# mapbox/robosat

Measured on AMD Instinct MI355X. Metric: 512x512 tiles/sec train+predict, 1/2/4/8 MI355X; mIoU vs CPU ref, higher is better.
Workload: dtype f32; 1 GPU; rs predict ResNet50-UNet, bs=16 3x512x512 fp32 per GPU, 2 classes (BASELINE configs[1]); parallelism=tiles sharded over 1 rank(s), no collective

## Files before the change

robosat_amd/csrc/conv_wino33_f32.hip:

```cpp
#define RS_CONV_INSTANTIATE
#include "conv_igemm_dma_kernel.h"
#include "final_head.h"

namespace {

struct Wino33Args {
  const float* src;
  const float* u;
  const float* scale;
  const float* shift;
  float* out;
  int N, H, W, Cin, Cout;
  int BBY, BBX;
  int nsub;
  int ncb;
  int relu;
  const float* hw;
  const float* hb;
  const double* hanchors;
  float* hout;
  unsigned char* hq;
  int hC, hmode, hov;
  float* stats;
  const float* mask;
  const unsigned char* mask_bits;
  const float* bn_y;
  const float* bn_mean;
  const float* bn_invstd;
};

typedef float f32x2 __attribute__((ext_vector_type(2)));
__device__ __forceinline__ f32x2 pk_add(f32x2 a, f32x2 b) {
  f32x2 d;
  asm("v_pk_add_f32 %0, %1, %2" : "=v"(d) : "v"(a), "v"(b));
  return d;
}
__device__ __forceinline__ f32x2 pk_sub(f32x2 a, f32x2 b) {
  f32x2 d;
  asm("v_pk_add_f32 %0, %1, %2 neg_lo:[0,1] neg_hi:[0,1]" : "=v"(d) : "v"(a), "v"(b));
  return d;
}
constexpr int kPB = 8, kHW = 2 * kPB + 2, kPITCH = kHW, kHALF = kHW / 2;
constexpr int kSBROWS = (kHW * kPITCH + 7) / 8 * 8;

__device__ __forceinline__ int w33_lane_tile(int l) { return (l & 1) | (((l >> 1) & 1) << 2) | (((l >> 2) & 1) << 1) | (l & 8); }
__device__ __forceinline__ int w33_swz(int row) { return (row ^ (row >> 1)) & 3; }

template <int TG, int CG, int MODE = 0>
__global__ __launch_bounds__(512, 1) void conv_wino33_f32_kernel(const Wino33Args p) {
  constexpr int HEAD = (MODE >= 1 && MODE <= 3) ? MODE : 0;
  constexpr bool BWD = MODE == 5;
  constexpr bool STATS = MODE == 4 || BWD;
  constexpr int NW = TG * CG;
  static_assert(NW == 8, "8 waves");
  static_assert(!HEAD || (TG == 4 && CG == 2), "the fused head: one 8x8 patch of tiles x all 32 couts per block");
  constexpr int BMT = 16 * TG, BN = 16 * CG;
  constexpr int SB = BMT / (kPB * kPB);
  static_assert(SB * kPB * kPB == BMT, "whole sub-blocks per block");
  constexpr int AROWS = SB * kSBROWS;
  constexpr int IA = (AROWS + 15) / 16, IB = 16 * BN / 16;
  constexpr int AROWS_PAD = IA * 16;
  constexpr int NI = (IA + IB + NW - 1) / NW;
  constexpr int STAGE = (AROWS_PAD + 16 * BN) * 64;
  constexpr int KC = 16;

  constexpr int HEADW = kHeadMaxC * 32 + kHeadMaxC, XROW = 4 * kHeadMaxC + 4, XCH = BMT * XROW;
  constexpr int XST = 2 * TG * BN;
  __shared__ __attribute__((aligned(16))) unsigned char smem[2 * STAGE + 2 * AROWS_PAD * 4 + (HEAD ? (HEADW + 2 * XCH) * 4 : 0) + (STATS ? 2 * XST * 4 : 0)];
  int* tabs = reinterpret_cast<int*>(smem + 2 * STAGE);
  float* hws = reinterpret_cast<float*>(smem + 2 * STAGE + 2 * AROWS_PAD * 4);
  float* xch = hws + HEADW;
  float* xst = reinterpret_cast<float*>(smem + 2 * STAGE + 2 * AROWS_PAD * 4);

  const int tid = threadIdx.x, lane = tid & 63;
  const int wave = __builtin_amdgcn_readfirstlane(tid >> 6);
  const int tg = wave % TG, cg = wave / TG;
  const int per_img = p.BBY * p.BBX;
  const int nk = p.Cin / KC;
  const int ntiles = ((p.nsub + SB - 1) / SB) * p.ncb;
  const int first = rs_xcd_remap(blockIdx.x, gridDim.x);
  const int nitems = (ntiles - first + (int)gridDim.x - 1) / (int)gridDim.x;
  const unsigned int lds0 = __builtin_amdgcn_readfirstlane(rs_lds_addr(smem));
  const long img = (long)p.H * p.W * p.Cin;

  auto decode = [&](int it, int& mblk, int& nblk) __attribute__((always_inline)) {
    mblk = it / p.ncb;
    nblk = it - mblk * p.ncb;
  };
  auto build_table = [&](int seq) __attribute__((always_inline)) {
    int mblk, nblk;
    decode(first + seq * (int)gridDim.x, mblk, nblk);
    const int sub0 = mblk * SB, nfirst = sub0 / per_img;
    int* tab = tabs + (seq & 1) * AROWS_PAD;
    for (int rho = tid; rho < AROWS_PAD; rho += 64 * NW) {
      int v = -1;
      if (rho < AROWS) {
        const int sb = rho / kSBROWS, rem = rho - sb * kSBROWS;
        const int hy = rem / kPITCH, xs = rem - hy * kPITCH;
        const int hx = hy >= kHW ? -1 : (xs < kHALF ? 2 * xs : 2 * (xs - kHALF) + 1);
        const int sub = sub0 + sb;
        if (hx >= 0 && sub < p.nsub) {
          const int n = sub / per_img, r2 = sub - n * per_img;
          const int bby = r2 / p.BBX, bbx = r2 - bby * p.BBX;
          const int y = 2 * bby * kPB - 1 + hy, x = 2 * bbx * kPB - 1 + hx;
          if ((unsigned)y < (unsigned)p.H && (unsigned)x < (unsigned)p.W) v = ((n - nfirst) * p.H + y) * p.W + x;
        }
      }
      tab[rho] = v;
    }
    rs_lds_writes_done();
  };

  const int ra = lane >> 2, pp = lane & 3;
  int doff[NI];
  int f_seq = 0, f_kc = 0, f_g = 0;
  __amdgpu_buffer_rsrc_t rsrc = rs_dma_rsrc<kDmaClamp>(p.src, 0);
  const __amdgpu_buffer_rsrc_t rsrcu = rs_dma_rsrc<kDmaClamp>(p.u, (long)16 * p.Cout * p.Cin * 4);
  auto fetch_item = [&]() __attribute__((always_inline)) {
    int mblk, nblk;
    decode(first + f_seq * (int)gridDim.x, mblk, nblk);
    const int nfirst = __builtin_amdgcn_readfirstlane((mblk * SB) / per_img);
    rsrc = rs_dma_rsrc<kDmaClamp>(p.src + nfirst * img, (long)(p.N - nfirst) * img * 4);
    const int* tab = tabs + (f_seq & 1) * AROWS_PAD;
#pragma unroll
    for (int j = 0; j < NI; ++j) {
      const int ii = wave + NW * j;
      if (ii < IA) {
        const int rho = 16 * ii + ra;
        const int pix = tab[rho];
        doff[j] = pix < 0 ? kDmaOOB : pix * (p.Cin * 4) + ((pp ^ w33_swz(rho)) & 3) * 16;
      } else {
        const int w = 16 * (ii - IA) + ra;
        const int xi = w / BN, co = w - xi * BN;
        doff[j] = ((xi * p.Cout + nblk * BN + co) * p.Cin) * 4 + ((pp ^ w33_swz(w)) & 3) * 16;
      }
    }
  };
  auto fetch_chunk = [&](auto interleave, bool past) __attribute__((always_inline)) {
    if (!past && f_kc == 0) fetch_item();
    const unsigned int fL = lds0 + (f_g & 1) * STAGE;
    const int fs = f_kc * KC * 4;
    interleave([&](int j) __attribute__((always_inline)) {
      const int ii = wave + NW * j;
      if (ii < IA) rs_dma16(rsrc, fL + ii * 1024, doff[j], fs);
      else if (ii < IA + IB) rs_dma16(rsrcu, fL + ii * 1024, doff[j], fs);
    });
    ++f_g;
    if (!past && ++f_kc == nk) {
      f_kc = 0;
      ++f_seq;
    }
  };

  const int l15 = lane & 15, pc = lane >> 4;
  const int t = 16 * tg + w33_lane_tile(l15);
  const int tsb = t / (kPB * kPB), tq = t - tsb * (kPB * kPB);
  const int tty = tq / kPB, ttx = tq - tty * kPB;
  int addrA[4][4];
  {
    const int rho0 = tsb * kSBROWS + 2 * tty * kPITCH + ttx;
#pragma unroll
    for (int r = 0; r < 4; ++r)
#pragma unroll
      for (int c = 0; c < 4; ++c) {
        const int rho = rho0 + r * kPITCH + (c >> 1) + (c & 1) * kHALF;
        addrA[r][c] = rho * 64 + ((pc ^ w33_swz(rho)) & 3) * 16;
      }
  }
  const int addrB = AROWS_PAD * 64 + (16 * cg + l15) * 64 + ((pc ^ w33_swz(l15)) & 3) * 16;

  if constexpr (HEAD) {
    for (int f = threadIdx.x; f < HEADW; f += 64 * NW) {
      const int c = f < kHeadMaxC * 32 ? f / 32 : f - kHeadMaxC * 32;
      hws[f] = c >= p.hC ? 0.f : (f < kHeadMaxC * 32 ? p.hw[f] : (p.hb ? p.hb[c] : 0.f));
    }
  }
  build_table(0);
  __syncthreads();
  fetch_chunk([&](auto issue) __attribute__((always_inline)) {
#pragma unroll
    for (int j = 0; j < NI; ++j) issue(j);
  }, false);
  const int total = nitems * nk;

  float hmine[kHeadMaxC];
  long hpix = -1;
  int hbuf = 0;
  auto finish_head = [&]() __attribute__((always_inline)) {
    if constexpr (HEAD) {
      if (cg == 0) {
        const float* xrow = xch + hbuf * XCH + (16 * tg + l15) * XROW + pc * kHeadMaxC;
        const f32x4 o0 = *reinterpret_cast<const f32x4*>(xrow), o1 = *reinterpret_cast<const f32x4*>(xrow + 4);
        float lg[kHeadMaxC];
#pragma unroll
        for (int c = 0; c < kHeadMaxC; ++c) lg[c] = (hmine[c] + (c < 4 ? o0[c] : o1[c - 4])) + hws[kHeadMaxC * 32 + c];
        if (hpix >= 0)
          rs_final_epilogue_rt(lg, p.hC, hpix, (long)p.H * p.W, HEAD == 1 ? (p.hmode & 1) : HEAD, p.hanchors, p.hq, p.hout, p.W, p.hov);
      }
    }
  };

  int st_buf = 0, st_row = 0, st_col = 0;
  auto finish_stats = [&]() __attribute__((always_inline)) {
    if constexpr (STATS) {
      if ((!BWD || p.stats) && threadIdx.x < 2 * BN) {
        const int which = threadIdx.x / BN, c = threadIdx.x - which * BN;
        const float* x = xst + st_buf * XST + which * TG * BN + c;
        float a = 0.f;
#pragma unroll
        for (int t = 0; t < TG; ++t) a += x[t * BN];
        p.stats[((long)st_row * 2 + which) * p.Cout + st_col + c] = a;
      }
    }
  };
  int g = 0;
  for (int seq = 0; seq < nitems; ++seq) {
    f32x4 acc[16];
#pragma unroll
    for (int x = 0; x < 16; ++x) acc[x] = f32x4{0.f, 0.f, 0.f, 0.f};

    for (int kc = 0; kc < nk; ++kc, ++g) {
      rs_dma_wait();
      __syncthreads();
      if (HEAD && kc == 0 && seq > 0) finish_head();
      if (STATS && kc == 0 && seq > 0) finish_stats();
      const unsigned char* L = smem + (g & 1) * STAGE;
      f32x4 V[16];
      {
        f32x2 Pl[4][4], Ph[4][4];
#pragma unroll
        for (int r = 0; r < 4; ++r)
#pragma unroll
          for (int c = 0; c < 4; ++c) {
            const f32x4 q = *reinterpret_cast<const f32x4*>(L + addrA[r][c]);
            Pl[r][c] = f32x2{q[0], q[1]};
            Ph[r][c] = f32x2{q[2], q[3]};
          }
        f32x2 Tl[4][4], Th[4][4];
#pragma unroll
        for (int r = 0; r < 4; ++r) {
          Tl[r][0] = pk_sub(Pl[r][0], Pl[r][2]);
          Tl[r][1] = pk_add(Pl[r][1], Pl[r][2]);
          Tl[r][2] = pk_sub(Pl[r][2], Pl[r][1]);
          Tl[r][3] = pk_sub(Pl[r][1], Pl[r][3]);
          Th[r][0] = pk_sub(Ph[r][0], Ph[r][2]);
          Th[r][1] = pk_add(Ph[r][1], Ph[r][2]);
          Th[r][2] = pk_sub(Ph[r][2], Ph[r][1]);
          Th[r][3] = pk_sub(Ph[r][1], Ph[r][3]);
        }
#pragma unroll
        for (int c = 0; c < 4; ++c) {
          const f32x2 l0 = pk_sub(Tl[0][c], Tl[2][c]), l1 = pk_add(Tl[1][c], Tl[2][c]), l2 = pk_sub(Tl[2][c], Tl[1][c]), l3 = pk_sub(Tl[1][c], Tl[3][c]);
          const f32x2 h0 = pk_sub(Th[0][c], Th[2][c]), h1 = pk_add(Th[1][c], Th[2][c]), h2 = pk_sub(Th[2][c], Th[1][c]), h3 = pk_sub(Th[1][c], Th[3][c]);
          V[0 * 4 + c] = f32x4{l0[0], l0[1], h0[0], h0[1]};
          V[1 * 4 + c] = f32x4{l1[0], l1[1], h1[0], h1[1]};
          V[2 * 4 + c] = f32x4{l2[0], l2[1], h2[0], h2[1]};
          V[3 * 4 + c] = f32x4{l3[0], l3[1], h3[0], h3[1]};
        }
      }
      const bool more = g + 1 < total;
      constexpr int NMMA = 64, PSTEP = NMMA / NI >= 1 ? NMMA / NI : 1;
      f32x4 Bq[16];
      Bq[0] = *reinterpret_cast<const f32x4*>(L + addrB);
      __builtin_amdgcn_sched_barrier(0);
      auto mfmas = [&](auto issue) __attribute__((always_inline)) {
#pragma unroll
        for (int x = 0; x < 16; ++x) {
          if (x + 1 < 16) {
            Bq[x + 1] = *reinterpret_cast<const f32x4*>(L + addrB + (x + 1) * BN * 64);
            __builtin_amdgcn_sched_barrier(0);
          }
#pragma unroll
          for (int k = 0; k < 4; ++k) {
            const int q = x * 4 + k;
            if (q % PSTEP == 0 && q / PSTEP < NI) issue(q / PSTEP);
            acc[x] = __builtin_amdgcn_mfma_f32_16x16x4f32(Bq[x][k], V[x][k], acc[x], 0, 0, 0);
          }
        }
      };
      fetch_chunk([&](auto issue) __attribute__((always_inline)) { mfmas(issue); }, !more);
      if (kc == 0 && seq + 1 < nitems) build_table(seq + 1);
    }

    int mblk, nblk;
    decode(first + seq * (int)gridDim.x, mblk, nblk);
    const int sub = mblk * SB + tsb;
    const bool live = sub < p.nsub;
    const int n = sub / per_img, r2 = sub - n * per_img;
    const int bby = r2 / p.BBX, bbx = r2 - bby * p.BBX;
    const int a0 = 2 * (bby * kPB + tty), b0 = 2 * (bbx * kPB + ttx);
    const int co = nblk * BN + 16 * cg + 4 * pc;
    f32x4 Y[2][2];
    if (live || HEAD) {
      f32x4 sc = {1.f, 1.f, 1.f, 1.f}, sh = {0.f, 0.f, 0.f, 0.f};
      if (p.scale) sc = *reinterpret_cast<const f32x4*>(p.scale + co);
      if (p.shift) sh = *reinterpret_cast<const f32x4*>(p.shift + co);
      f32x4 R[2][4];
#pragma unroll
      for (int b = 0; b < 4; ++b) {
        R[0][b] = (acc[0 * 4 + b] + acc[1 * 4 + b]) + acc[2 * 4 + b];
        R[1][b] = (acc[1 * 4 + b] - acc[2 * 4 + b]) - acc[3 * 4 + b];
      }
#pragma unroll
      for (int u = 0; u < 2; ++u)
#pragma unroll
        for (int v = 0; v < 2; ++v) {
          f32x4 y = v == 0 ? (R[u][0] + R[u][1]) + R[u][2] : (R[u][1] - R[u][2]) - R[u][3];
          y = y * sc + sh;
          if (p.relu) {
#pragma unroll
            for (int e = 0; e < 4; ++e) y[e] = fmaxf(y[e], 0.f);
          }
          Y[u][v] = y;
        }
    }
    if constexpr (!HEAD) {
      f32x4 s0 = {0.f, 0.f, 0.f, 0.f}, s1 = {0.f, 0.f, 0.f, 0.f};
      if (live) {
        if constexpr (BWD) {
          long o[4];
          bool ok[4];
          f32x4 zm[4], yv[4];
          unsigned int bits[4];
#pragma unroll
          for (int q = 0; q < 4; ++q) {
            const int a = a0 + (q >> 1), b = b0 + (q & 1);
            ok[q] = a < p.H && b < p.W;
            o[q] = ok[q] ? ((long)(n * p.H + a) * p.W + b) * p.Cout + co : (long)co;
          }
          if (p.mask) {
#pragma unroll
            for (int q = 0; q < 4; ++q) zm[q] = *reinterpret_cast<const f32x4*>(p.mask + o[q]);
          }
          if (p.mask_bits) {
#pragma unroll
            for (int q = 0; q < 4; ++q) bits[q] = p.mask_bits[o[q] >> 3];
          }
          f32x4 mu = {0.f, 0.f, 0.f, 0.f}, is = mu;
          if (p.stats) {
#pragma unroll
            for (int q = 0; q < 4; ++q) yv[q] = *reinterpret_cast<const f32x4*>(p.bn_y + o[q]);
            mu = *reinterpret_cast<const f32x4*>(p.bn_mean + co);
            is = *reinterpret_cast<const f32x4*>(p.bn_invstd + co);
          }
#pragma unroll
          for (int q = 0; q < 4; ++q) {
            f32x4 y = Y[q >> 1][q & 1];
            if (p.mask) {
#pragma unroll
              for (int e = 0; e < 4; ++e) y[e] = zm[q][e] > 0.f ? y[e] : 0.f;
            }
            if (p.mask_bits) {
              const unsigned int nib = bits[q] >> (o[q] & 4);
#pragma unroll
              for (int e = 0; e < 4; ++e) y[e] = ((nib >> e) & 1u) ? y[e] : 0.f;
            }
            if (!ok[q]) continue;
            *reinterpret_cast<f32x4*>(p.out + o[q]) = y;
            if (p.stats) {
              s0 += y;
              s1 += y * ((yv[q] - mu) * is);
            }
          }
        } else {
#pragma unroll
          for (int u = 0; u < 2; ++u)
#pragma unroll
            for (int v = 0; v < 2; ++v) {
              const int a = a0 + u, b = b0 + v;
              if (a >= p.H || b >= p.W) continue;
              *reinterpret_cast<f32x4*>(p.out + ((long)(n * p.H + a) * p.W + b) * p.Cout + co) = Y[u][v];
              if constexpr (STATS) {
                s0 += Y[u][v];
                s1 += Y[u][v] * Y[u][v];
              }
            }
        }
      }
      if constexpr (STATS) {
        if (!BWD || p.stats) {
#pragma unroll
          for (int e = 0; e < 4; ++e) {
            s0[e] = rs_row16_sum(s0[e]);
            s1[e] = rs_row16_sum(s1[e]);
          }
          st_buf = seq & 1;
          st_row = mblk;
          st_col = nblk * BN;
          if (l15 == 0) {
            float* x = xst + st_buf * XST + tg * BN + 16 * cg + 4 * pc;
            *reinterpret_cast<f32x4*>(x) = s0;
            *reinterpret_cast<f32x4*>(x + TG * BN) = s1;
            rs_lds_writes_done();
          }
        }
      }
    } else {
      float part[4][kHeadMaxC];
#pragma unroll
      for (int c = 0; c < kHeadMaxC; ++c) {
        if (c < p.hC) {
          const f32x4 wv = *reinterpret_cast<const f32x4*>(hws + c * 32 + 16 * cg + 4 * pc);
#pragma unroll
          for (int px = 0; px < 4; ++px) {
            const f32x4 y = Y[px >> 1][px & 1];
            float v = fmaf(y[3], wv[3], fmaf(y[2], wv[2], fmaf(y[1], wv[1], y[0] * wv[0])));
            v = rs_xor32_sum(rs_xor16_sum(v));
            part[px][c] = v;
          }
        } else {
#pragma unroll
          for (int px = 0; px < 4; ++px) part[px][c] = 0.f;
        }
      }
      hbuf = seq & 1;
      if (cg == 1 && pc == 0) {
        float* xrow = xch + hbuf * XCH + (16 * tg + l15) * XROW;
#pragma unroll
        for (int px = 0; px < 4; ++px) {
          *reinterpret_cast<f32x4*>(xrow + px * kHeadMaxC) = f32x4{part[px][0], part[px][1], part[px][2], part[px][3]};
          *reinterpret_cast<f32x4*>(xrow + px * kHeadMaxC + 4) = f32x4{part[px][4], part[px][5], part[px][6], part[px][7]};
        }
        rs_lds_writes_done();
      }
#pragma unroll
      for (int c = 0; c < kHeadMaxC; ++c) hmine[c] = pc == 0 ? part[0][c] : (pc == 1 ? part[1][c] : (pc == 2 ? part[2][c] : part[3][c]));
      const int a = a0 + (pc >> 1), b = b0 + (pc & 1);
      hpix = (live && a < p.H && b < p.W) ? (long)(n * p.H + a) * p.W + b : -1;
    }
  }
  if constexpr (HEAD) {
    __syncthreads();
    if (nitems > 0) finish_head();
  }
  if constexpr (STATS) {
    __syncthreads();
    if (nitems > 0) finish_stats();
  }
  rs_dma_wait();
}

__global__ void pack_wino33_weight_kernel(const float* __restrict__ w, float* __restrict__ u, int Cout, int Cin, long total) {
  const long i = (long)blockIdx.x * blockDim.x + threadIdx.x;
  if (i >= total) return;
  const int ci = (int)(i % Cin), co = (int)(i / Cin);
  const float* g = w + (long)co * 9 * Cin + ci;
  float gg[3][3];
#pragma unroll
  for (int r = 0; r < 3; ++r)
#pragma unroll
    for (int c = 0; c < 3; ++c) gg[r][c] = g[(long)(r * 3 + c) * Cin];
  float t[4][3];
#pragma unroll
  for (int c = 0; c < 3; ++c) {
    t[0][c] = gg[0][c];
    t[1][c] = 0.5f * ((gg[0][c] + gg[1][c]) + gg[2][c]);
    t[2][c] = 0.5f * ((gg[0][c] - gg[1][c]) + gg[2][c]);
    t[3][c] = gg[2][c];
  }
#pragma unroll
  for (int r = 0; r < 4; ++r) {
    const float v[4] = {t[r][0], 0.5f * ((t[r][0] + t[r][1]) + t[r][2]), 0.5f * ((t[r][0] - t[r][1]) + t[r][2]), t[r][2]};
#pragma unroll
    for (int c = 0; c < 4; ++c) u[((long)(r * 4 + c) * Cout + co) * Cin + ci] = v[c];
  }
}

int w33_plan(const rs_conv_desc* d, int* cgroups) {
  if (!d || d->N <= 0 || d->Hs <= 0 || d->Ws <= 0 || d->C1 < 32 || (d->C1 % 16) || d->C2 != 0 || d->Cout <= 0 || (d->Cout % 16)) return 0;
  if (!(d->ups == 0 && d->kh == 3 && d->kw == 3 && d->stride == 1 && d->pad == 1 && d->Ho == d->Hs && d->Wo == d->Ws && !d->stem)) return 0;
  if ((d->Hs + 1) / 2 < kPB || (d->Ws + 1) / 2 < kPB) return 0;
  *cgroups = (d->Cout % 32 == 0) ? 2 : 1;
  const int sb = 16 * (8 / *cgroups) / (kPB * kPB);
  if ((long)(sb + 1) * d->Hs * d->Ws * d->C1 * 4 >= (1L << 31)) return 0;
  if ((long)16 * d->Cout * d->C1 * 4 >= (1L << 31)) return 0;
  if ((long)d->N * d->Ho * d->Wo * d->Cout >= (1L << 62)) return 0;
  return 1;
}

}

extern "C" int rs_conv2d_wino33_ok(const rs_conv_desc* d) {
  int cgn;
  return w33_plan(d, &cgn);
}

extern "C" const char* rs_conv2d_wino33_name(const rs_conv_desc* d) {
  int cgn;
  if (!w33_plan(d, &cgn)) return "";
  return cgn == 2 ? "conv_wino_f32<3x3,p8,64x32>" : "conv_wino_f32<3x3,p8,128x16>";
}

extern "C" int rs_conv2d_wino33_head_ok(const rs_conv_desc* d, int C) {
  int cgn;
  return w33_plan(d, &cgn) && cgn == 2 && d->Cout == 32 && C >= 1 && C <= kHeadMaxC;
}

extern "C" const char* rs_conv2d_wino33_head_name(void) { return "conv_wino_f32<3x3+final,p8,64x32>"; }

extern "C" int rs_pack_wino33_weight(const float* w_krsc, float* u, int Cout, int Cin, rs_stream_t stream) {
  if (!w_krsc || !u || Cout <= 0 || Cin <= 0) return RS_EINVAL;
  const long total = (long)Cout * Cin;
  pack_wino33_weight_kernel<<<rs_cdiv(total, 256), 256, 0, (hipStream_t)stream>>>(w_krsc, u, Cout, Cin, total);
  return RS_LAUNCH_RESULT();
}

extern "C" int rs_conv2d_fwd_wino33(const rs_conv_desc* d, const float* src, const float* u, const float* scale, const float* shift,
                                    float* out, rs_stream_t stream) {
  int cgn;
  if (!w33_plan(d, &cgn) || !src || !u || !out) return RS_EINVAL;
  Wino33Args a;
  a.src = src;
  a.u = u;
  a.scale = scale;
  a.shift = shift;
  a.out = out;
  a.N = d->N;
  a.H = d->Hs;
  a.W = d->Ws;
  a.Cin = d->C1;
  a.Cout = d->Cout;
  a.BBY = rs_cdiv((d->Hs + 1) / 2, kPB);
  a.BBX = rs_cdiv((d->Ws + 1) / 2, kPB);
  a.nsub = d->N * a.BBY * a.BBX;
  a.ncb = d->Cout / (16 * cgn);
  a.relu = d->relu;
  a.hw = a.hb = nullptr;
  a.hanchors = nullptr;
  a.hout = nullptr;
  a.hq = nullptr;
  a.hC = a.hmode = a.hov = 0;
  a.stats = nullptr;
  a.mask = a.bn_y = a.bn_mean = a.bn_invstd = nullptr;
  a.mask_bits = nullptr;
  const int sb = 16 * (8 / cgn) / (kPB * kPB);
  const long items = (long)rs_cdiv(a.nsub, sb) * a.ncb;
  if (items >= (1L << 31)) return RS_EINVAL;
  const int grid = (int)(items < rs_cu_count() ? items : rs_cu_count());
  hipStream_t s = (hipStream_t)stream;
  if (cgn == 2) conv_wino33_f32_kernel<4, 2><<<grid, 512, 0, s>>>(a);
  else conv_wino33_f32_kernel<8, 1><<<grid, 512, 0, s>>>(a);
  return RS_LAUNCH_RESULT();
}

extern "C" int rs_conv2d_fwd_wino33_head(const rs_conv_desc* d, const float* src, const float* u, const float* scale, const float* shift,
                                         const float* final_w, const float* final_b, int C, int mode, const double* anchors,
                                         int overlap, float* out, uint8_t* qout, rs_stream_t stream) {
  if (!rs_conv2d_wino33_head_ok(d, C) || !src || !u || !final_w || mode < 0 || mode > 3) return RS_EINVAL;
  if (mode <= 1 ? !out : !qout) return RS_EINVAL;
  if (mode == 2 && (!anchors || C < 2 || overlap < 0 || 2 * overlap >= d->Hs || 2 * overlap >= d->Ws)) return RS_EINVAL;
  if (mode == 3 && C < 2) return RS_EINVAL;
  Wino33Args a;
  a.src = src;
  a.u = u;
  a.scale = scale;
  a.shift = shift;
  a.out = nullptr;
  a.N = d->N;
  a.H = d->Hs;
  a.W = d->Ws;
  a.Cin = d->C1;
  a.Cout = d->Cout;
  a.BBY = rs_cdiv((d->Hs + 1) / 2, kPB);
  a.BBX = rs_cdiv((d->Ws + 1) / 2, kPB);
  a.nsub = d->N * a.BBY * a.BBX;
  a.ncb = 1;
  a.relu = d->relu;
  a.hw = final_w;
  a.hb = final_b;
  a.hanchors = anchors;
  a.hout = out;
  a.hq = qout;
  a.hC = C;
  a.hmode = mode;
  a.hov = overlap;
  a.stats = nullptr;
  a.mask = a.bn_y = a.bn_mean = a.bn_invstd = nullptr;
  a.mask_bits = nullptr;
  const long items = a.nsub;
  if (items >= (1L << 31)) return RS_EINVAL;
  const int grid = (int)(items < rs_cu_count() ? items : rs_cu_count());
  hipStream_t s = (hipStream_t)stream;
  if (mode <= 1) conv_wino33_f32_kernel<4, 2, 1><<<grid, 512, 0, s>>>(a);
  else if (mode == 2) conv_wino33_f32_kernel<4, 2, 2><<<grid, 512, 0, s>>>(a);
  else conv_wino33_f32_kernel<4, 2, 3><<<grid, 512, 0, s>>>(a);
  return RS_LAUNCH_RESULT();
}

extern "C" long rs_conv2d_wino33_stats_rows(const rs_conv_desc* d) {
  int cgn;
  if (!w33_plan(d, &cgn)) return RS_EINVAL;
  const int sb = 16 * (8 / cgn) / (kPB * kPB);
  return rs_cdiv((long)d->N * rs_cdiv((d->Hs + 1) / 2, kPB) * rs_cdiv((d->Ws + 1) / 2, kPB), sb);
}

extern "C" int rs_conv2d_fwd_wino33_stats(const rs_conv_desc* d, const float* src, const float* u, float* out, float* stats,
                                          rs_stream_t stream) {
  int cgn;
  if (!w33_plan(d, &cgn) || !src || !u || !out || !stats) return RS_EINVAL;
  Wino33Args a;
  a.src = src;
  a.u = u;
  a.scale = a.shift = nullptr;
  a.out = out;
  a.N = d->N;
  a.H = d->Hs;
  a.W = d->Ws;
  a.Cin = d->C1;
  a.Cout = d->Cout;
  a.BBY = rs_cdiv((d->Hs + 1) / 2, kPB);
  a.BBX = rs_cdiv((d->Ws + 1) / 2, kPB);
  a.nsub = d->N * a.BBY * a.BBX;
  a.ncb = d->Cout / (16 * cgn);
  a.relu = 0;
  a.hw = a.hb = nullptr;
  a.hanchors = nullptr;
  a.hout = nullptr;
  a.hq = nullptr;
  a.hC = a.hmode = a.hov = 0;
  a.stats = stats;
  a.mask = a.bn_y = a.bn_mean = a.bn_invstd = nullptr;
  a.mask_bits = nullptr;
  const int sb = 16 * (8 / cgn) / (kPB * kPB);
  const long items = (long)rs_cdiv(a.nsub, sb) * a.ncb;
  if (items >= (1L << 31)) return RS_EINVAL;
  const int grid = (int)(items < rs_cu_count() ? items : rs_cu_count());
  hipStream_t s = (hipStream_t)stream;
  if (cgn == 2) conv_wino33_f32_kernel<4, 2, 4><<<grid, 512, 0, s>>>(a);
  else conv_wino33_f32_kernel<8, 1, 4><<<grid, 512, 0, s>>>(a);
  return RS_LAUNCH_RESULT();
}

extern "C" int rs_conv2d_dgrad_wino33(const rs_conv_desc* d, const float* dy, const float* u, const float* mask, const uint8_t* mask_bits,
                                      const float* bn_y, const float* bn_mean, const float* bn_invstd, float* out, float* stats,
                                      rs_stream_t stream) {
  int cgn;
  if (!w33_plan(d, &cgn) || cgn != 2 || !dy || !u || !out) return RS_EINVAL;
  if (mask && mask_bits) return RS_EINVAL;
  if (mask_bits && (d->Cout % 8) != 0) return RS_EINVAL;
  if (stats ? (!bn_y || !bn_mean || !bn_invstd) : (bn_y || bn_mean || bn_invstd)) return RS_EINVAL;
  Wino33Args a;
  a.src = dy;
  a.u = u;
  a.scale = a.shift = nullptr;
  a.out = out;
  a.N = d->N;
  a.H = d->Hs;
  a.W = d->Ws;
  a.Cin = d->C1;
  a.Cout = d->Cout;
  a.BBY = rs_cdiv((d->Hs + 1) / 2, kPB);
  a.BBX = rs_cdiv((d->Ws + 1) / 2, kPB);
  a.nsub = d->N * a.BBY * a.BBX;
  a.ncb = d->Cout / (16 * cgn);
  a.relu = 0;
  a.hw = a.hb = nullptr;
  a.hanchors = nullptr;
  a.hout = nullptr;
  a.hq = nullptr;
  a.hC = a.hmode = a.hov = 0;
  a.stats = stats;
  a.mask = mask;
  a.mask_bits = mask_bits;
  a.bn_y = bn_y;
  a.bn_mean = bn_mean;
  a.bn_invstd = bn_invstd;
  const int sb = 16 * (8 / cgn) / (kPB * kPB);
  const long items = (long)rs_cdiv(a.nsub, sb) * a.ncb;
  if (items >= (1L << 31)) return RS_EINVAL;
  const int grid = (int)(items < rs_cu_count() ? items : rs_cu_count());
  hipStream_t s = (hipStream_t)stream;
  conv_wino33_f32_kernel<4, 2, 5><<<grid, 512, 0, s>>>(a);
  return RS_LAUNCH_RESULT();
}
```

robosat_amd/csrc/final_head.h:

```cpp
#pragma once
#include "common.h"

constexpr int kHeadMaxC = 8;

__device__ __forceinline__ void rs_final_epilogue_rt(float (&acc)[kHeadMaxC], int C, long pix, long HW, int softmax,
                                                     const double* __restrict__ anchors, uint8_t* __restrict__ qout,
                                                     float* __restrict__ out, int Wimg, int ov) {
  if (softmax == 1 || softmax == 2) {
    float mx = acc[0];
#pragma unroll
    for (int c = 1; c < kHeadMaxC; ++c)
      if (c < C) mx = fmaxf(mx, acc[c]);
    float sum = 0.f;
#pragma unroll
    for (int c = 0; c < kHeadMaxC; ++c)
      if (c < C) {
        acc[c] = expf(acc[c] - mx);
        sum += acc[c];
      }
#pragma unroll
    for (int c = 0; c < kHeadMaxC; ++c)
      if (c < C) acc[c] = acc[c] / sum;
  }
  const long n = pix / HW, hw = pix - n * HW;
  if (softmax == 2) {
    if (C < 2) return;
    const int Himg = (int)(HW / Wimg);
    const int yy = (int)(hw / Wimg), xx = (int)(hw - (long)yy * Wimg);
    const int S_h = Himg - 2 * ov, S_w = Wimg - 2 * ov;
    if (yy < ov || yy >= Himg - ov || xx < ov || xx >= Wimg - ov) return;
    uint8_t* qo = qout + ((n * S_h + (yy - ov)) * (long)S_w + (xx - ov)) * (C - 1);
#pragma unroll
    for (int c = 1; c < kHeadMaxC; ++c)
      if (c < C) {
        const double pf = (double)acc[c];
        int q = (int)(pf * 255.0);
        q = q < 0 ? 0 : (q > 255 ? 255 : q);
        while (q < 255 && anchors[q + 1] <= pf) ++q;
        while (q >= 0 && anchors[q] > pf) --q;
        qo[c - 1] = (uint8_t)((q + 1) & 0xff);
      }
    return;
  }
  if (softmax == 3) {
    int best = 0;
    float bv = acc[0];
#pragma unroll
    for (int c = 1; c < kHeadMaxC; ++c)
      if (c < C && acc[c] > bv) {
        bv = acc[c];
        best = c;
      }
    qout[pix] = (uint8_t)best;
    return;
  }
  float* o = out + n * C * HW + hw;
#pragma unroll
  for (int c = 0; c < kHeadMaxC; ++c)
    if (c < C) o[c * HW] = acc[c];
}
```

Before: 1657 tiles/s.

## Specialise fused head on class count and incrementalise item decode in Winograd conv

Templates the fused final-head Winograd kernel on a compile-time class bound (2/4/8) so the 2-class predict path carries fewer head registers, less LDS and smaller exchange traffic. It also replaces the per-item integer divisions used to decode tile indices with an incrementally advanced Item state, hoists per-thread table geometry and the weight DMA offsets out of the loop, and makes the DMA offsets scalar. The epilogue now takes (n,y,x) instead of a flat pixel index, which removes long divisions. The cost is more template instantiations and more complex item bookkeeping. That bookkeeping could break if SB or the grid stride assumptions change.

```diff
diff --git a/robosat_amd/csrc/conv_wino33_f32.hip b/robosat_amd/csrc/conv_wino33_f32.hip
--- a/robosat_amd/csrc/conv_wino33_f32.hip
+++ b/robosat_amd/csrc/conv_wino33_f32.hip
@@ -46,9 +46,10 @@
 __device__ __forceinline__ int w33_lane_tile(int l) { return (l & 1) | (((l >> 1) & 1) << 2) | (((l >> 2) & 1) << 1) | (l & 8); }
 __device__ __forceinline__ int w33_swz(int row) { return (row ^ (row >> 1)) & 3; }
 
-template <int TG, int CG, int MODE = 0>
+template <int TG, int CG, int MODE = 0, int HC = kHeadMaxC>
 __global__ __launch_bounds__(512, 1) void conv_wino33_f32_kernel(const Wino33Args p) {
   constexpr int HEAD = (MODE >= 1 && MODE <= 3) ? MODE : 0;
+  static_assert(HC == 2 || HC == 4 || HC == 8, "class bound of the fused head");
   constexpr bool BWD = MODE == 5;
   constexpr bool STATS = MODE == 4 || BWD;
   constexpr int NW = TG * CG;
@@ -57,6 +58,7 @@
   constexpr int BMT = 16 * TG, BN = 16 * CG;
   constexpr int SB = BMT / (kPB * kPB);
   static_assert(SB * kPB * kPB == BMT, "whole sub-blocks per block");
+  static_assert(SB == 1 || SB == 2, "the item state below: one or two sub-blocks");
   constexpr int AROWS = SB * kSBROWS;
   constexpr int IA = (AROWS + 15) / 16, IB = 16 * BN / 16;
   constexpr int AROWS_PAD = IA * 16;
@@ -64,7 +66,7 @@
   constexpr int STAGE = (AROWS_PAD + 16 * BN) * 64;
   constexpr int KC = 16;
 
-  constexpr int HEADW = kHeadMaxC * 32 + kHeadMaxC, XROW = 4 * kHeadMaxC + 4, XCH = BMT * XROW;
+  constexpr int HEADW = HC * 32 + (HC + 3) / 4 * 4, XROW = 4 * HC + 4, XCH = BMT * XROW;
   constexpr int XST = 2 * TG * BN;
   __shared__ __attribute__((aligned(16))) unsigned char smem[2 * STAGE + 2 * AROWS_PAD * 4 + (HEAD ? (HEADW + 2 * XCH) * 4 : 0) + (STATS ? 2 * XST * 4 : 0)];
   int* tabs = reinterpret_cast<int*>(smem + 2 * STAGE);
@@ -83,67 +85,117 @@
   const unsigned int lds0 = __builtin_amdgcn_readfirstlane(rs_lds_addr(smem));
   const long img = (long)p.H * p.W * p.Cin;
 
-  auto decode = [&](int it, int& mblk, int& nblk) __attribute__((always_inline)) {
-    mblk = it / p.ncb;
-    nblk = it - mblk * p.ncb;
+  struct Item {
+    int mblk, nblk, nfirst;
+    int n[SB], y0[SB], x0[SB], nb[SB];
+    bool live[SB];
   };
-  auto build_table = [&](int seq) __attribute__((always_inline)) {
-    int mblk, nblk;
-    decode(first + seq * (int)gridDim.x, mblk, nblk);
-    const int sub0 = mblk * SB, nfirst = sub0 / per_img;
+  const int uni_first = __builtin_amdgcn_readfirstlane(first), uni_grid = __builtin_amdgcn_readfirstlane((int)gridDim.x);
+  int d_mblk = uni_first / p.ncb, d_nblk = uni_first - d_mblk * p.ncb;
+  const int dq = uni_grid / p.ncb, dr = uni_grid - dq * p.ncb;
+  auto decode_next = [&](Item& s) __attribute__((always_inline)) {
+    s.mblk = d_mblk;
+    s.nblk = d_nblk;
+    const int sub0 = d_mblk * SB;
+    int n = __builtin_amdgcn_readfirstlane(sub0 / per_img);
+    const int r2 = sub0 - n * per_img;
+    int bby = __builtin_amdgcn_readfirstlane(r2 / p.BBX);
+    int bbx = r2 - bby * p.BBX;
+    s.nfirst = n;
+#pragma unroll
+    for (int sb = 0; sb < SB; ++sb) {
+      s.live[sb] = sub0 + sb < p.nsub;
+      s.n[sb] = n;
+      s.y0[sb] = 2 * bby * kPB - 1;
+      s.x0[sb] = 2 * bbx * kPB - 1;
+      s.nb[sb] = (n - s.nfirst) * p.H;
+      if (++bbx == p.BBX) {
+        bbx = 0;
+        if (++bby == p.BBY) {
+          bby = 0;
+          ++n;
+        }
+      }
+    }
+    d_mblk += dq;
+    d_nblk += dr;
+    if (d_nblk >= p.ncb) {
+      d_nblk -= p.ncb;
+      ++d_mblk;
+    }
+  };
+  Item cur, nxt;
+  decode_next(cur);
+  nxt = cur;
+
+  constexpr int NT = (AROWS_PAD + 64 * NW - 1) / (64 * NW);
+  int t_hy[NT], t_hx[NT];
+  bool t_sb[NT];
+#pragma unroll
+  for (int e = 0; e < NT; ++e) {
+    const int rho = tid + 64 * NW * e;
+    const int sb = rho / kSBROWS, rem = rho - sb * kSBROWS;
+    const int hy = rem / kPITCH, xs = rem - hy * kPITCH;
+    const bool halo = rho < AROWS && hy < kHW;
+    t_sb[e] = sb > 0 && sb < SB;
+    t_hy[e] = halo ? hy : -(1 << 24);
+    t_hx[e] = xs < kHALF ? 2 * xs : 2 * (xs - kHALF) + 1;
+  }
+  auto build_table = [&](const Item& s, int seq) __attribute__((always_inline)) {
     int* tab = tabs + (seq & 1) * AROWS_PAD;
-    for (int rho = tid; rho < AROWS_PAD; rho += 64 * NW) {
-      int v = -1;
-      if (rho < AROWS) {
-        const int sb = rho / kSBROWS, rem = rho - sb * kSBROWS;
-        const int hy = rem / kPITCH, xs = rem - hy * kPITCH;
-        const int hx = hy >= kHW ? -1 : (xs < kHALF ? 2 * xs : 2 * (xs - kHALF) + 1);
-        const int sub = sub0 + sb;
-        if (hx >= 0 && sub < p.nsub) {
-          const int n = sub / per_img, r2 = sub - n * per_img;
-          const int bby = r2 / p.BBX, bbx = r2 - bby * p.BBX;
-          const int y = 2 * bby * kPB - 1 + hy, x = 2 * bbx * kPB - 1 + hx;
-          if ((unsigned)y < (unsigned)p.H && (unsigned)x < (unsigned)p.W) v = ((n - nfirst) * p.H + y) * p.W + x;
-        }
-      }
-      tab[rho] = v;
+#pragma unroll
+    for (int e = 0; e < NT; ++e) {
+      const int rho = tid + 64 * NW * e;
+      if (rho < AROWS_PAD) {
+        const bool one = SB > 1 && t_sb[e];
+        const int y = (one ? s.y0[SB - 1] : s.y0[0]) + t_hy[e], x = (one ? s.x0[SB - 1] : s.x0[0]) + t_hx[e];
+        const bool in = (one ? s.live[SB - 1] : s.live[0]) && (unsigned)y < (unsigned)p.H && (unsigned)x < (unsigned)p.W;
+        tab[rho] = in ? ((one ? s.nb[SB - 1] : s.nb[0]) + y) * p.W + x : -1;
+      }
     }
     rs_lds_writes_done();
   };
 
   const int ra = lane >> 2, pp = lane & 3;
   int doff[NI];
-  int f_seq = 0, f_kc = 0, f_g = 0;
+#pragma unroll
+  for (int j = 0; j < NI; ++j) {
+    const int ii = wave + NW * j;
+    static_assert((BN & (BN - 1)) == 0, "BN: a power of two");
+    const unsigned int w = 16u * (unsigned int)(ii - IA) + ra;
+    const int xi = (int)(w / BN), co = (int)(w % BN);
+    doff[j] = ii < IA ? kDmaOOB : ((xi * p.Cout + co) * p.Cin) * 4 + ((pp ^ w33_swz((int)w)) & 3) * 16;
+  }
+  int f_seq = 0, f_kc = 0, f_g = 0, f_nb = 0;
   __amdgpu_buffer_rsrc_t rsrc = rs_dma_rsrc<kDmaClamp>(p.src, 0);
   const __amdgpu_buffer_rsrc_t rsrcu = rs_dma_rsrc<kDmaClamp>(p.u, (long)16 * p.Cout * p.Cin * 4);
-  auto fetch_item = [&]() __attribute__((always_inline)) {
-    int mblk, nblk;
-    decode(first + f_seq * (int)gridDim.x, mblk, nblk);
-    const int nfirst = __builtin_amdgcn_readfirstlane((mblk * SB) / per_img);
-    rsrc = rs_dma_rsrc<kDmaClamp>(p.src + nfirst * img, (long)(p.N - nfirst) * img * 4);
+  auto fetch_item = [&](const Item& s) __attribute__((always_inline)) {
+    rsrc = rs_dma_rsrc<kDmaClamp>(p.src + s.nfirst * img, (long)(p.N - s.nfirst) * img * 4);
+    f_nb = s.nblk * BN * p.Cin * 4;
     const int* tab = tabs + (f_seq & 1) * AROWS_PAD;
+    int pix[NI];
 #pragma unroll
     for (int j = 0; j < NI; ++j) {
       const int ii = wave + NW * j;
-      if (ii < IA) {
+      if (NW * j < IA) pix[j] = tab[16 * (ii < IA ? ii : IA - 1) + ra];
+    }
+#pragma unroll
+    for (int j = 0; j < NI; ++j) {
+      const int ii = wave + NW * j;
+      if (NW * j < IA && ii < IA) {
         const int rho = 16 * ii + ra;
-        const int pix = tab[rho];
-        doff[j] = pix < 0 ? kDmaOOB : pix * (p.Cin * 4) + ((pp ^ w33_swz(rho)) & 3) * 16;
-      } else {
-        const int w = 16 * (ii - IA) + ra;
-        const int xi = w / BN, co = w - xi * BN;
-        doff[j] = ((xi * p.Cout + nblk * BN + co) * p.Cin) * 4 + ((pp ^ w33_swz(w)) & 3) * 16;
+        doff[j] = pix[j] < 0 ? kDmaOOB : pix[j] * (p.Cin * 4) + ((pp ^ w33_swz(rho)) & 3) * 16;
       }
     }
   };
   auto fetch_chunk = [&](auto interleave, bool past) __attribute__((always_inline)) {
-    if (!past && f_kc == 0) fetch_item();
+    if (!past && f_kc == 0) fetch_item(nxt);
     const unsigned int fL = lds0 + (f_g & 1) * STAGE;
-    const int fs = f_kc * KC * 4;
+    const int fs = __builtin_amdgcn_readfirstlane(f_kc * KC * 4), fsu = __builtin_amdgcn_readfirstlane(fs + f_nb);
     interleave([&](int j) __attribute__((always_inline)) {
       const int ii = wave + NW * j;
       if (ii < IA) rs_dma16(rsrc, fL + ii * 1024, doff[j], fs);
-      else if (ii < IA + IB) rs_dma16(rsrcu, fL + ii * 1024, doff[j], fs);
+      else if (ii < IA + IB) rs_dma16(rsrcu, fL + ii * 1024, doff[j], fsu);
     });
     ++f_g;
     if (!past && ++f_kc == nk) {
@@ -154,7 +206,7 @@
 
   const int l15 = lane & 15, pc = lane >> 4;
   const int t = 16 * tg + w33_lane_tile(l15);
-  const int tsb = t / (kPB * kPB), tq = t - tsb * (kPB * kPB);
+  const int tsb = 16 * tg / (kPB * kPB), tq = t - tsb * (kPB * kPB);
   const int tty = tq / kPB, ttx = tq - tty * kPB;
   int addrA[4][4];
   {
@@ -171,11 +223,11 @@
 
   if constexpr (HEAD) {
     for (int f = threadIdx.x; f < HEADW; f += 64 * NW) {
-      const int c = f < kHeadMaxC * 32 ? f / 32 : f - kHeadMaxC * 32;
-      hws[f] = c >= p.hC ? 0.f : (f < kHeadMaxC * 32 ? p.hw[f] : (p.hb ? p.hb[c] : 0.f));
-    }
-  }
-  build_table(0);
+      const int c = f < HC * 32 ? f / 32 : f - HC * 32;
+      hws[f] = c >= p.hC ? 0.f : (f < HC * 32 ? p.hw[f] : (p.hb ? p.hb[c] : 0.f));
+    }
+  }
+  build_table(cur, 0);
   __syncthreads();
   fetch_chunk([&](auto issue) __attribute__((always_inline)) {
 #pragma unroll
@@ -183,19 +235,31 @@
   }, false);
   const int total = nitems * nk;
 
-  float hmine[kHeadMaxC];
-  long hpix = -1;
+  float hmine[HC];
+  int hn = -1, hpy = 0, hpx = 0;
   int hbuf = 0;
   auto finish_head = [&]() __attribute__((always_inline)) {
     if constexpr (HEAD) {
       if (cg == 0) {
-        const float* xrow = xch + hbuf * XCH + (16 * tg + l15) * XROW + pc * kHeadMaxC;
-        const f32x4 o0 = *reinterpret_cast<const f32x4*>(xrow), o1 = *reinterpret_cast<const f32x4*>(xrow + 4);
-        float lg[kHeadMaxC];
-#pragma unroll
-        for (int c = 0; c < kHeadMaxC; ++c) lg[c] = (hmine[c] + (c < 4 ? o0[c] : o1[c - 4])) + hws[kHeadMaxC * 32 + c];
-        if (hpix >= 0)
-          rs_final_epilogue_rt(lg, p.hC, hpix, (long)p.H * p.W, HEAD == 1 ? (p.hmode & 1) : HEAD, p.hanchors, p.hq, p.hout, p.W, p.hov);
+        const float* xrow = xch + hbuf * XCH + (16 * tg + l15) * XROW + pc * HC;
+        float o[HC];
+        if constexpr (HC == 2) {
+          const f32x2 v = *reinterpret_cast<const f32x2*>(xrow);
+          o[0] = v[0];
+          o[1] = v[1];
+        } else {
+#pragma unroll
+          for (int q = 0; q < HC / 4; ++q) {
+            const f32x4 v = *reinterpret_cast<const f32x4*>(xrow + 4 * q);
+#pragma unroll
+            for (int e = 0; e < 4; ++e) o[4 * q + e] = v[e];
+          }
+        }
+        float lg[HC];
+#pragma unroll
+        for (int c = 0; c < HC; ++c) lg[c] = (hmine[c] + o[c]) + hws[HC * 32 + c];
+        if (hn >= 0)
+          rs_final_epilogue_rt<HC>(lg, p.hC, hn, hpy, hpx, p.H, p.W, HEAD == 1 ? (p.hmode & 1) : HEAD, p.hanchors, p.hq, p.hout, p.hov);
       }
     }
   };
@@ -279,17 +343,19 @@
         }
       };
       fetch_chunk([&](auto issue) __attribute__((always_inline)) { mfmas(issue); }, !more);
-      if (kc == 0 && seq + 1 < nitems) build_table(seq + 1);
-    }
-
-    int mblk, nblk;
-    decode(first + seq * (int)gridDim.x, mblk, nblk);
-    const int sub = mblk * SB + tsb;
-    const bool live = sub < p.nsub;
-    const int n = sub / per_img, r2 = sub - n * per_img;
-    const int bby = r2 / p.BBX, bbx = r2 - bby * p.BBX;
-    const int a0 = 2 * (bby * kPB + tty), b0 = 2 * (bbx * kPB + ttx);
+      if (kc == 0 && seq + 1 < nitems) {
+        decode_next(nxt);
+        build_table(nxt, seq + 1);
+      }
+    }
+
+    const int mblk = cur.mblk, nblk = cur.nblk;
+    const bool one = SB > 1 && tsb > 0;
+    const bool live = one ? cur.live[SB - 1] : cur.live[0];
+    const int n = one ? cur.n[SB - 1] : cur.n[0];
+    const int a0 = (one ? cur.y0[SB - 1] : cur.y0[0]) + 1 + 2 * tty, b0 = (one ? cur.x0[SB - 1] : cur.x0[0]) + 1 + 2 * ttx;
     const int co = nblk * BN + 16 * cg + 4 * pc;
+    cur = nxt;
     f32x4 Y[2][2];
     if (live || HEAD) {
       f32x4 sc = {1.f, 1.f, 1.f, 1.f}, sh = {0.f, 0.f, 0.f, 0.f};
@@ -396,10 +462,10 @@
         }
       }
     } else {
-      float part[4][kHeadMaxC];
-#pragma unroll
-      for (int c = 0; c < kHeadMaxC; ++c) {
-        if (c < p.hC) {
+      float part[4][HC];
+#pragma unroll
+      for (int c = 0; c < HC; ++c) {
+        if (c <= HC / 2 || c < p.hC) {
           const f32x4 wv = *reinterpret_cast<const f32x4*>(hws + c * 32 + 16 * cg + 4 * pc);
 #pragma unroll
           for (int px = 0; px < 4; ++px) {
@@ -418,15 +484,21 @@
         float* xrow = xch + hbuf * XCH + (16 * tg + l15) * XROW;
 #pragma unroll
         for (int px = 0; px < 4; ++px) {
-          *reinterpret_cast<f32x4*>(xrow + px * kHeadMaxC) = f32x4{part[px][0], part[px][1], part[px][2], part[px][3]};
-          *reinterpret_cast<f32x4*>(xrow + px * kHeadMaxC + 4) = f32x4{part[px][4], part[px][5], part[px][6], part[px][7]};
+          if constexpr (HC == 2) {
+            *reinterpret_cast<f32x2*>(xrow + px * HC) = f32x2{part[px][0], part[px][1]};
+          } else {
+#pragma unroll
+            for (int q = 0; q < HC / 4; ++q)
+              *reinterpret_cast<f32x4*>(xrow + px * HC + 4 * q) = f32x4{part[px][4 * q], part[px][4 * q + 1], part[px][4 * q + 2], part[px][4 * q + 3]};
+          }
         }
         rs_lds_writes_done();
       }
 #pragma unroll
-      for (int c = 0; c < kHeadMaxC; ++c) hmine[c] = pc == 0 ? part[0][c] : (pc == 1 ? part[1][c] : (pc == 2 ? part[2][c] : part[3][c]));
-      const int a = a0 + (pc >> 1), b = b0 + (pc & 1);
-      hpix = (live && a < p.H && b < p.W) ? (long)(n * p.H + a) * p.W + b : -1;
+      for (int c = 0; c < HC; ++c) hmine[c] = pc == 0 ? part[0][c] : (pc == 1 ? part[1][c] : (pc == 2 ? part[2][c] : part[3][c]));
+      hpy = a0 + (pc >> 1);
+      hpx = b0 + (pc & 1);
+      hn = (live && hpy < p.H && hpx < p.W) ? n : -1;
     }
   }
   if constexpr (HEAD) {
@@ -581,9 +653,16 @@
   if (items >= (1L << 31)) return RS_EINVAL;
   const int grid = (int)(items < rs_cu_count() ? items : rs_cu_count());
   hipStream_t s = (hipStream_t)stream;
-  if (mode <= 1) conv_wino33_f32_kernel<4, 2, 1><<<grid, 512, 0, s>>>(a);
-  else if (mode == 2) conv_wino33_f32_kernel<4, 2, 2><<<grid, 512, 0, s>>>(a);
-  else conv_wino33_f32_kernel<4, 2, 3><<<grid, 512, 0, s>>>(a);
+#define RS_W33_HEAD(MODE)                                                          \
+  do {                                                                             \
+    if (C <= 2) conv_wino33_f32_kernel<4, 2, MODE, 2><<<grid, 512, 0, s>>>(a);      \
+    else if (C <= 4) conv_wino33_f32_kernel<4, 2, MODE, 4><<<grid, 512, 0, s>>>(a); \
+    else conv_wino33_f32_kernel<4, 2, MODE, 8><<<grid, 512, 0, s>>>(a);             \
+  } while (0)
+  if (mode <= 1) RS_W33_HEAD(1);
+  else if (mode == 2) RS_W33_HEAD(2);
+  else RS_W33_HEAD(3);
+#undef RS_W33_HEAD
   return RS_LAUNCH_RESULT();
 }
 
diff --git a/robosat_amd/csrc/final_head.h b/robosat_amd/csrc/final_head.h
--- a/robosat_amd/csrc/final_head.h
+++ b/robosat_amd/csrc/final_head.h
@@ -3,35 +3,35 @@
 
 constexpr int kHeadMaxC = 8;
 
-__device__ __forceinline__ void rs_final_epilogue_rt(float (&acc)[kHeadMaxC], int C, long pix, long HW, int softmax,
+template <int HC>
+__device__ __forceinline__ void rs_final_epilogue_rt(float (&acc)[HC], int C, int n, int yy, int xx, int Himg, int Wimg, int softmax,
                                                      const double* __restrict__ anchors, uint8_t* __restrict__ qout,
-                                                     float* __restrict__ out, int Wimg, int ov) {
+                                                     float* __restrict__ out, int ov) {
+  static_assert(HC >= 1 && HC <= kHeadMaxC, "at most kHeadMaxC classes");
   if (softmax == 1 || softmax == 2) {
     float mx = acc[0];
 #pragma unroll
-    for (int c = 1; c < kHeadMaxC; ++c)
+    for (int c = 1; c < HC; ++c)
       if (c < C) mx = fmaxf(mx, acc[c]);
     float sum = 0.f;
 #pragma unroll
-    for (int c = 0; c < kHeadMaxC; ++c)
+    for (int c = 0; c < HC; ++c)
       if (c < C) {
         acc[c] = expf(acc[c] - mx);
         sum += acc[c];
       }
 #pragma unroll
-    for (int c = 0; c < kHeadMaxC; ++c)
+    for (int c = 0; c < HC; ++c)
       if (c < C) acc[c] = acc[c] / sum;
   }
-  const long n = pix / HW, hw = pix - n * HW;
+  const long HW = (long)Himg * Wimg, hw = (long)yy * Wimg + xx;
   if (softmax == 2) {
     if (C < 2) return;
-    const int Himg = (int)(HW / Wimg);
-    const int yy = (int)(hw / Wimg), xx = (int)(hw - (long)yy * Wimg);
     const int S_h = Himg - 2 * ov, S_w = Wimg - 2 * ov;
     if (yy < ov || yy >= Himg - ov || xx < ov || xx >= Wimg - ov) return;
-    uint8_t* qo = qout + ((n * S_h + (yy - ov)) * (long)S_w + (xx - ov)) * (C - 1);
+    uint8_t* qo = qout + (((long)n * S_h + (yy - ov)) * (long)S_w + (xx - ov)) * (C - 1);
 #pragma unroll
-    for (int c = 1; c < kHeadMaxC; ++c)
+    for (int c = 1; c < HC; ++c)
       if (c < C) {
         const double pf = (double)acc[c];
         int q = (int)(pf * 255.0);
@@ -46,16 +46,16 @@
     int best = 0;
     float bv = acc[0];
 #pragma unroll
-    for (int c = 1; c < kHeadMaxC; ++c)
+    for (int c = 1; c < HC; ++c)
       if (c < C && acc[c] > bv) {
         bv = acc[c];
         best = c;
       }
-    qout[pix] = (uint8_t)best;
+    qout[(long)n * HW + hw] = (uint8_t)best;
     return;
   }
-  float* o = out + n * C * HW + hw;
+  float* o = out + (long)n * C * HW + hw;
 #pragma unroll
-  for (int c = 0; c < kHeadMaxC; ++c)
+  for (int c = 0; c < HC; ++c)
     if (c < C) o[c * HW] = acc[c];
 }
```

After: 1675 tiles/s (median of 6 runs). 1.1% higher.
